# filrg/split_learning

Hardware: AMD Instinct MI355X
Metric: images/sec (whole node) VGG16/CIFAR10 cut=7 (higher is better)
Workload: dtype fp32; 1 GPU; model=VGG16_CIFAR10, global_batch=32, image=3x32x32, cut_layer=7, optimizer=SGD(lr=5e-4, momentum=0.5), control_count=1, mode=serial-recompute, parallelism=split2 x dp1

## Files before the change

### split_learning_amd/ops/csrc/wino.hip

```cpp
#include "torch_util.h"

namespace slk {

template <bool FLIP>
__global__ void wino_wt_kernel(const float* __restrict__ w,
                               float* __restrict__ U, int Cw0, int Cw1) {
  const long total = (long)Cw0 * Cw1;
  const long tstride = (long)gridDim.x * blockDim.x;
  for (long e = (long)blockIdx.x * blockDim.x + threadIdx.x; e < 4 * total;
       e += tstride) {
    const int a = (int)(e & 3);
    const long i = e >> 2;
    const int cols = FLIP ? Cw0 : Cw1;
    const int c = (int)(i % cols);
    const int r = (int)(i / cols);
    const int co = FLIP ? c : r;
    const int ci = FLIP ? r : c;
    float t[3];
    #pragma unroll
    for (int b = 0; b < 3; ++b) {
      const float g0 = w[(((long)co * Cw1 + ci) * 3 + (FLIP ? 2 : 0)) * 3 +
                         (FLIP ? 2 - b : b)];
      const float g1 = w[(((long)co * Cw1 + ci) * 3 + 1) * 3 +
                         (FLIP ? 2 - b : b)];
      const float g2 = w[(((long)co * Cw1 + ci) * 3 + (FLIP ? 0 : 2)) * 3 +
                         (FLIP ? 2 - b : b)];
      t[b] = a == 0 ? g0
           : a == 1 ? 0.5f * (g0 + g1 + g2)
           : a == 2 ? 0.5f * (g0 - g1 + g2)
           : g2;
    }
    U[((long)(a * 4 + 0) * total) + i] = t[0];
    U[((long)(a * 4 + 1) * total) + i] = 0.5f * (t[0] + t[1] + t[2]);
    U[((long)(a * 4 + 2) * total) + i] = 0.5f * (t[0] - t[1] + t[2]);
    U[((long)(a * 4 + 3) * total) + i] = t[2];
  }
}

__global__ void wino_in_kernel(const float* __restrict__ x,
                               float* __restrict__ V, int B, int Ci, int H,
                               int W, int tH, int tW, int pad, FastDiv d_T,
                               FastDiv d_thw, FastDiv d_tw) {
  const int T = B * tH * tW;
  const long total = (long)Ci * T;
  const long stride = (long)gridDim.x * blockDim.x;
  for (long i = (long)blockIdx.x * blockDim.x + threadIdx.x; i < total;
       i += stride) {
    const unsigned cc = d_T.div((unsigned)i);
    const unsigned t = d_T.mod((unsigned)i, cc);
    const unsigned b = d_thw.div(t);
    const unsigned rem = d_thw.mod(t, b);
    const unsigned th = d_tw.div(rem);
    const unsigned tw = d_tw.mod(rem, th);
    const int ih0 = (int)th * 2 - pad;
    const int iw0 = (int)tw * 2 - pad;
    const float* xp = x + ((long)b * Ci + cc) * H * W;
    float d[4][4];
    #pragma unroll
    for (int a = 0; a < 4; ++a) {
      const int ih = ih0 + a;
      const bool hv = (unsigned)ih < (unsigned)H;
      #pragma unroll
      for (int bb = 0; bb < 4; ++bb) {
        const int iw = iw0 + bb;
        const bool v = hv && (unsigned)iw < (unsigned)W;
        d[a][bb] = v ? xp[(long)ih * W + iw] : 0.f;
      }
    }
    float u[4][4];
    #pragma unroll
    for (int bb = 0; bb < 4; ++bb) {
      u[0][bb] = d[0][bb] - d[2][bb];
      u[1][bb] = d[1][bb] + d[2][bb];
      u[2][bb] = d[2][bb] - d[1][bb];
      u[3][bb] = d[1][bb] - d[3][bb];
    }
    #pragma unroll
    for (int a = 0; a < 4; ++a) {
      const float v0 = u[a][0] - u[a][2];
      const float v1 = u[a][1] + u[a][2];
      const float v2 = u[a][2] - u[a][1];
      const float v3 = u[a][1] - u[a][3];
      V[((long)(a * 4 + 0) * Ci + cc) * T + t] = v0;
      V[((long)(a * 4 + 1) * Ci + cc) * T + t] = v1;
      V[((long)(a * 4 + 2) * Ci + cc) * T + t] = v2;
      V[((long)(a * 4 + 3) * Ci + cc) * T + t] = v3;
    }
  }
}

__global__ void wino_out_kernel(const float* __restrict__ Mm,
                                float* __restrict__ y,
                                const float* __restrict__ bias, int B, int Co,
                                int OH, int OW, int tH, int tW, FastDiv d_T,
                                FastDiv d_thw, FastDiv d_tw) {
  const int T = B * tH * tW;
  const long total = (long)Co * T;
  const long stride = (long)gridDim.x * blockDim.x;
  for (long i = (long)blockIdx.x * blockDim.x + threadIdx.x; i < total;
       i += stride) {
    const unsigned co = d_T.div((unsigned)i);
    const unsigned t = d_T.mod((unsigned)i, co);
    const unsigned b = d_thw.div(t);
    const unsigned rem = d_thw.mod(t, b);
    const unsigned th = d_tw.div(rem);
    const unsigned tw = d_tw.mod(rem, th);
    float m[4][4];
    #pragma unroll
    for (int f = 0; f < 16; ++f)
      m[f >> 2][f & 3] = Mm[((long)f * Co + co) * T + t];
    float u[2][4];
    #pragma unroll
    for (int bb = 0; bb < 4; ++bb) {
      u[0][bb] = m[0][bb] + m[1][bb] + m[2][bb];
      u[1][bb] = m[1][bb] - m[2][bb] - m[3][bb];
    }
    const float bv = bias != nullptr ? bias[co] : 0.f;
    float* yp = y + ((long)b * Co + co) * OH * OW + (long)th * 2 * OW + tw * 2;
    yp[0] = u[0][0] + u[0][1] + u[0][2] + bv;
    yp[1] = u[0][1] - u[0][2] - u[0][3] + bv;
    yp[OW] = u[1][0] + u[1][1] + u[1][2] + bv;
    yp[OW + 1] = u[1][1] - u[1][2] - u[1][3] + bv;
  }
}

__global__ void wino_gyA_kernel(const float* __restrict__ gy,
                                float* __restrict__ Wg, int B, int Co, int OH,
                                int OW, int tH, int tW, FastDiv d_T,
                                FastDiv d_thw, FastDiv d_tw) {
  const int T = B * tH * tW;
  const long total = (long)Co * T;
  const long stride = (long)gridDim.x * blockDim.x;
  for (long i = (long)blockIdx.x * blockDim.x + threadIdx.x; i < total;
       i += stride) {
    const unsigned co = d_T.div((unsigned)i);
    const unsigned t = d_T.mod((unsigned)i, co);
    const unsigned b = d_thw.div(t);
    const unsigned rem = d_thw.mod(t, b);
    const unsigned th = d_tw.div(rem);
    const unsigned tw = d_tw.mod(rem, th);
    const float* gp = gy + ((long)b * Co + co) * OH * OW
                      + (long)th * 2 * OW + tw * 2;
    const float g00 = gp[0], g01 = gp[1], g10 = gp[OW], g11 = gp[OW + 1];
    float r0c0 = g00, r0c1 = g01;
    float r1c0 = g00 + g10, r1c1 = g01 + g11;
    float r2c0 = g00 - g10, r2c1 = g01 - g11;
    float r3c0 = -g10, r3c1 = -g11;
    #pragma unroll
    for (int a = 0; a < 4; ++a) {
      const float c0 = a == 0 ? r0c0 : a == 1 ? r1c0 : a == 2 ? r2c0 : r3c0;
      const float c1 = a == 0 ? r0c1 : a == 1 ? r1c1 : a == 2 ? r2c1 : r3c1;
      Wg[((long)(a * 4 + 0) * Co + co) * T + t] = c0;
      Wg[((long)(a * 4 + 1) * Co + co) * T + t] = c0 + c1;
      Wg[((long)(a * 4 + 2) * Co + co) * T + t] = c0 - c1;
      Wg[((long)(a * 4 + 3) * Co + co) * T + t] = -c1;
    }
  }
}

__global__ void wino_gw_kernel(const float* __restrict__ dU,
                               float* __restrict__ gw, int Co, int Ci) {
  const long total = (long)Co * Ci;
  const long stride = (long)gridDim.x * blockDim.x;
  for (long i = (long)blockIdx.x * blockDim.x + threadIdx.x; i < total;
       i += stride) {
    float u[4][4];
    #pragma unroll
    for (int f = 0; f < 16; ++f) u[f >> 2][f & 3] = dU[(long)f * total + i];
    float t[3][4];
    #pragma unroll
    for (int b = 0; b < 4; ++b) {
      t[0][b] = u[0][b] + 0.5f * (u[1][b] + u[2][b]);
      t[1][b] = 0.5f * (u[1][b] - u[2][b]);
      t[2][b] = 0.5f * (u[1][b] + u[2][b]) + u[3][b];
    }
    #pragma unroll
    for (int r = 0; r < 3; ++r) {
      gw[i * 9 + r * 3 + 0] = t[r][0] + 0.5f * (t[r][1] + t[r][2]);
      gw[i * 9 + r * 3 + 1] = 0.5f * (t[r][1] - t[r][2]);
      gw[i * 9 + r * 3 + 2] = 0.5f * (t[r][1] + t[r][2]) + t[r][3];
    }
  }
}

at::Tensor matmul_f32(const at::Tensor&, const at::Tensor&, bool, bool,
                      c10::optional<at::Tensor>, bool);

at::Tensor conv2d_wino(const at::Tensor& x, const at::Tensor& w,
                       c10::optional<at::Tensor> bias, int pad, bool flip) {
  TORCH_CHECK(x.is_cuda() && x.dim() == 4 && x.scalar_type() == at::kFloat);
  TORCH_CHECK(w.size(2) == 3 && w.size(3) == 3, "wino: 3x3 only");
  auto xc = x.contiguous();
  auto wc = w.contiguous();
  const int B = x.size(0), H = x.size(2), W = x.size(3);
  const int Co = flip ? w.size(1) : w.size(0);
  const int Ci = flip ? w.size(0) : w.size(1);
  TORCH_CHECK(x.size(1) == Ci, "wino: channel mismatch");
  const int OH = H + 2 * pad - 2, OW = W + 2 * pad - 2;
  TORCH_CHECK(OH % 2 == 0 && OW % 2 == 0, "wino: even output dims only");
  const int tH = OH / 2, tW = OW / 2;
  const int T = B * tH * tW;
  auto stream = c10::hip::getCurrentHIPStream().stream();

  auto U = at::empty({16, Co, Ci}, x.options());
  auto V = at::empty({16, Ci, T}, x.options());
  {
    const long tot = (long)Co * Ci * 4;
    const int grid = (int)std::min<long>((tot + 255) / 256, 4096);
    if (flip) {
      hipLaunchKernelGGL(wino_wt_kernel<true>, dim3(grid), dim3(256), 0,
                         stream, wc.data_ptr<float>(), U.data_ptr<float>(),
                         (int)w.size(0), (int)w.size(1));
    } else {
      hipLaunchKernelGGL(wino_wt_kernel<false>, dim3(grid), dim3(256), 0,
                         stream, wc.data_ptr<float>(), U.data_ptr<float>(),
                         (int)w.size(0), (int)w.size(1));
    }
  }
  {
    FastDiv d_T, d_thw, d_tw;
    d_T.init(T);
    d_thw.init(tH * tW);
    d_tw.init(tW);
    const long tot = (long)Ci * T;
    const int grid = (int)std::min<long>((tot + 255) / 256, 8192);
    hipLaunchKernelGGL(wino_in_kernel, dim3(grid), dim3(256), 0, stream,
                       xc.data_ptr<float>(), V.data_ptr<float>(), B, Ci, H, W,
                       tH, tW, pad, d_T, d_thw, d_tw);
  }
  auto Mm = matmul_f32(U, V, false, false, c10::nullopt, false);
  auto y = at::empty({B, Co, OH, OW}, x.options());
  {
    FastDiv d_T, d_thw, d_tw;
    d_T.init(T);
    d_thw.init(tH * tW);
    d_tw.init(tW);
    const long tot = (long)Co * T;
    const int grid = (int)std::min<long>((tot + 255) / 256, 8192);
    hipLaunchKernelGGL(wino_out_kernel, dim3(grid), dim3(256), 0, stream,
                       Mm.data_ptr<float>(), y.data_ptr<float>(),
                       bias.has_value() ? bias->data_ptr<float>() : nullptr,
                       B, Co, OH, OW, tH, tW, d_T, d_thw, d_tw);
  }
  return y;
}


constexpr int WF_CO = 32;
constexpr int WF_T = 32;
constexpr int WF_CK = 8;
constexpr int WF_ULD = WF_CO + 1;
constexpr int WF_VLD = WF_T + 1;

template <bool FLIP>
__global__ __launch_bounds__(256, 3) void wino_fused_kernel(
    const float* __restrict__ x, const float* __restrict__ w,
    const float* __restrict__ bias, float* __restrict__ y, int B, int Ci,
    int H, int W, int Co, int OH, int OW, int tH, int tW, int pad,
    int ci_per, int CW, FastDiv d_thw, FastDiv d_tw) {
  const int ci_begin = blockIdx.z * ci_per;
  const int ci_end = min(Ci, ci_begin + ci_per);
  __shared__ float Ul[16 * WF_CK * WF_ULD];
  __shared__ float Vl[16 * WF_CK * WF_VLD];

  const int T = B * tH * tW;
  const int co0 = blockIdx.y * WF_CO;
  const int t0 = blockIdx.x * WF_T;

  const int tid = threadIdx.x;
  const int lane = tid & 63;
  const int wid = tid >> 6;
  const int wco = (wid >> 1) * 16;
  const int wt = (wid & 1) * 16;
  const int frag_r = lane >> 4;
  const int frag_c = lane & 15;

  f32x4 acc[16];
  #pragma unroll
  for (int f = 0; f < 16; ++f) acc[f] = f32x4{};

  const int v_ci = tid >> 5;
  const int v_t = tid & 31;
  const int tg = t0 + v_t;
  const unsigned vb = d_thw.div((unsigned)tg);
  const unsigned vrem = d_thw.mod((unsigned)tg, vb);
  const unsigned vth = d_tw.div(vrem);
  const unsigned vtw = d_tw.mod(vrem, vth);
  const int ih0 = (int)vth * 2 - pad;
  const int iw0 = (int)vtw * 2 - pad;
  const long xplane = ((long)vb * Ci + v_ci) * H * W;
  const int w_co = tid >> 3;
  const int w_ci = tid & 7;

  float d[4][4];
  float wr[9];

  auto load_regs = [&](int ci0) {
    const float* xp = x + xplane + (long)ci0 * H * W;
    #pragma unroll
    for (int a = 0; a < 4; ++a) {
      const int ih = ih0 + a;
      const bool hv = (unsigned)ih < (unsigned)H;
      #pragma unroll
      for (int bb = 0; bb < 4; ++bb) {
        const int iw = iw0 + bb;
        const bool v = hv && (unsigned)iw < (unsigned)W;
        d[a][bb] = v ? xp[(long)ih * W + iw] : 0.f;
      }
    }
    const long wbase = FLIP
        ? ((long)(ci0 + w_ci) * CW + (co0 + w_co)) * 9
        : ((long)(co0 + w_co) * CW + (ci0 + w_ci)) * 9;
    #pragma unroll
    for (int k = 0; k < 9; ++k) wr[k] = w[wbase + (FLIP ? 8 - k : k)];
  };

  auto store_stage = [&]() {
    float u[4][4];
    #pragma unroll
    for (int bb = 0; bb < 4; ++bb) {
      u[0][bb] = d[0][bb] - d[2][bb];
      u[1][bb] = d[1][bb] + d[2][bb];
      u[2][bb] = d[2][bb] - d[1][bb];
      u[3][bb] = d[1][bb] - d[3][bb];
    }
    #pragma unroll
    for (int a = 0; a < 4; ++a) {
      Vl[((a * 4 + 0) * WF_CK + v_ci) * WF_VLD + v_t] = u[a][0] - u[a][2];
      Vl[((a * 4 + 1) * WF_CK + v_ci) * WF_VLD + v_t] = u[a][1] + u[a][2];
      Vl[((a * 4 + 2) * WF_CK + v_ci) * WF_VLD + v_t] = u[a][2] - u[a][1];
      Vl[((a * 4 + 3) * WF_CK + v_ci) * WF_VLD + v_t] = u[a][1] - u[a][3];
    }
    float t0[3], t1[3], t2[3], t3[3];
    #pragma unroll
    for (int bb = 0; bb < 3; ++bb) {
      const float g0 = wr[bb], g1 = wr[3 + bb], g2 = wr[6 + bb];
      t0[bb] = g0;
      t1[bb] = 0.5f * (g0 + g1 + g2);
      t2[bb] = 0.5f * (g0 - g1 + g2);
      t3[bb] = g2;
    }
    const float* tr[4] = {t0, t1, t2, t3};
    #pragma unroll
    for (int a = 0; a < 4; ++a) {
      const float* t = tr[a];
      Ul[((a * 4 + 0) * WF_CK + w_ci) * WF_ULD + w_co] = t[0];
      Ul[((a * 4 + 1) * WF_CK + w_ci) * WF_ULD + w_co] = 0.5f * (t[0] + t[1] + t[2]);
      Ul[((a * 4 + 2) * WF_CK + w_ci) * WF_ULD + w_co] = 0.5f * (t[0] - t[1] + t[2]);
      Ul[((a * 4 + 3) * WF_CK + w_ci) * WF_ULD + w_co] = t[2];
    }
  };

  load_regs(ci_begin);
  for (int ci0 = ci_begin; ci0 < ci_end; ci0 += WF_CK) {
    store_stage();
    __syncthreads();
    if (ci0 + WF_CK < ci_end) load_regs(ci0 + WF_CK);
    #pragma unroll
    for (int f = 0; f < 16; ++f) {
      #pragma unroll
      for (int kk = 0; kk < WF_CK / 4; ++kk) {
        const int kr = kk * 4 + frag_r;
        const float a = Ul[(f * WF_CK + kr) * WF_ULD + wco + frag_c];
        const float b = Vl[(f * WF_CK + kr) * WF_VLD + wt + frag_c];
        acc[f] = __builtin_amdgcn_mfma_f32_16x16x4f32(a, b, acc[f], 0, 0, 0);
      }
    }
    __syncthreads();
  }

  #pragma unroll
  for (int i = 0; i < 4; ++i) {
    const int co = co0 + wco + frag_r * 4 + i;
    const int t = t0 + wt + frag_c;
    if (co >= Co || t >= T) continue;
    float m[4][4];
    #pragma unroll
    for (int f = 0; f < 16; ++f) m[f >> 2][f & 3] = acc[f][i];
    float u0[4], u1[4];
    #pragma unroll
    for (int bb = 0; bb < 4; ++bb) {
      u0[bb] = m[0][bb] + m[1][bb] + m[2][bb];
      u1[bb] = m[1][bb] - m[2][bb] - m[3][bb];
    }
    const float bv = (bias != nullptr && blockIdx.z == 0) ? bias[co] : 0.f;
    const unsigned b = d_thw.div((unsigned)t);
    const unsigned rem = d_thw.mod((unsigned)t, b);
    const unsigned th = d_tw.div(rem);
    const unsigned tw = d_tw.mod(rem, th);
    float* yp = y + (long)blockIdx.z * B * Co * OH * OW +
                ((long)b * Co + co) * OH * OW + (long)th * 2 * OW + tw * 2;
    const float o00 = u0[0] + u0[1] + u0[2] + bv;
    const float o01 = u0[1] - u0[2] - u0[3] + bv;
    const float o10 = u1[0] + u1[1] + u1[2] + bv;
    const float o11 = u1[1] - u1[2] - u1[3] + bv;
    yp[0] = o00;
    yp[1] = o01;
    yp[OW] = o10;
    yp[OW + 1] = o11;
  }
}

at::Tensor conv2d_wino_bwdw(const at::Tensor& gy, const at::Tensor& x,
                            int pad) {
  TORCH_CHECK(gy.is_cuda() && x.is_cuda() && gy.dim() == 4 && x.dim() == 4);
  auto gyc = gy.contiguous();
  auto xc = x.contiguous();
  const int B = x.size(0), Ci = x.size(1), H = x.size(2), W = x.size(3);
  const int Co = gy.size(1), OH = gy.size(2), OW = gy.size(3);
  TORCH_CHECK(OH == H + 2 * pad - 2 && OW == W + 2 * pad - 2,
              "wino_bwdw geometry");
  TORCH_CHECK(OH % 2 == 0 && OW % 2 == 0, "wino_bwdw: even output dims only");
  const int tH = OH / 2, tW = OW / 2;
  const int T = B * tH * tW;
  auto stream = c10::hip::getCurrentHIPStream().stream();
  FastDiv d_T, d_thw, d_tw;
  d_T.init(T);
  d_thw.init(tH * tW);
  d_tw.init(tW);

  auto Wg = at::empty({16, Co, T}, x.options());
  auto Vx = at::empty({16, Ci, T}, x.options());
  {
    const long tot = (long)Co * T;
    const int grid = (int)std::min<long>((tot + 255) / 256, 8192);
    hipLaunchKernelGGL(wino_gyA_kernel, dim3(grid), dim3(256), 0, stream,
                       gyc.data_ptr<float>(), Wg.data_ptr<float>(), B, Co, OH,
                       OW, tH, tW, d_T, d_thw, d_tw);
  }
  {
    const long tot = (long)Ci * T;
    const int grid = (int)std::min<long>((tot + 255) / 256, 8192);
    hipLaunchKernelGGL(wino_in_kernel, dim3(grid), dim3(256), 0, stream,
                       xc.data_ptr<float>(), Vx.data_ptr<float>(), B, Ci, H, W,
                       tH, tW, pad, d_T, d_thw, d_tw);
  }
  auto dU = matmul_f32(Wg, Vx, false, true, c10::nullopt, false);
  auto gw = at::empty({Co, Ci, 3, 3}, x.options());
  {
    const long tot = (long)Co * Ci;
    const int grid = (int)std::min<long>((tot + 255) / 256, 4096);
    hipLaunchKernelGGL(wino_gw_kernel, dim3(grid), dim3(256), 0, stream,
                       dU.data_ptr<float>(), gw.data_ptr<float>(), Co, Ci);
  }
  return gw;
}

__global__ __launch_bounds__(256, 2) void wino_bwdw_fused_kernel(
    const float* __restrict__ gy, const float* __restrict__ x,
    float* __restrict__ slab, int B, int Ci, int H, int W, int Co, int OH,
    int OW, int tH, int tW, int pad, int t_per, FastDiv d_thw, FastDiv d_tw) {
  __shared__ float Gl[16 * 8 * 33];
  __shared__ float Xl[16 * 8 * 33];

  const int T = B * tH * tW;
  const int ci0 = blockIdx.y * 32;
  const int co0 = blockIdx.x * 32;
  const int t_begin = blockIdx.z * t_per;
  const int t_end = min(T, t_begin + t_per);

  const int tid = threadIdx.x;
  const int lane = tid & 63;
  const int wid = tid >> 6;
  const int wco = (wid >> 1) * 16;
  const int wci = (wid & 1) * 16;
  const int frag_r = lane >> 4;
  const int frag_c = lane & 15;

  f32x4 acc[16];
  #pragma unroll
  for (int f = 0; f < 16; ++f) acc[f] = f32x4{};

  const int s_ch = tid >> 3;
  const int s_t = tid & 7;

  float gg[2][2];
  float xd[4][4];

  auto load_regs = [&](int t0) {
    const int t = t0 + s_t;
    const int tc = t < T ? t : T - 1;
    const bool tv = t < t_end;
    const unsigned b = d_thw.div((unsigned)tc);
    const unsigned rem = d_thw.mod((unsigned)tc, b);
    const unsigned th = d_tw.div(rem);
    const unsigned tw = d_tw.mod(rem, th);
    {
      const float* gp = gy + ((long)b * Co + co0 + s_ch) * OH * OW
                        + (long)th * 2 * OW + tw * 2;
      gg[0][0] = tv ? gp[0] : 0.f;
      gg[0][1] = tv ? gp[1] : 0.f;
      gg[1][0] = tv ? gp[OW] : 0.f;
      gg[1][1] = tv ? gp[OW + 1] : 0.f;
    }
    {
      const int ih0 = (int)th * 2 - pad;
      const int iw0 = (int)tw * 2 - pad;
      const float* xp = x + ((long)b * Ci + ci0 + s_ch) * H * W;
      #pragma unroll
      for (int a = 0; a < 4; ++a) {
        const int ih = ih0 + a;
        const bool hv = tv && (unsigned)ih < (unsigned)H;
        #pragma unroll
        for (int bb = 0; bb < 4; ++bb) {
          const int iw = iw0 + bb;
          const bool v = hv && (unsigned)iw < (unsigned)W;
          xd[a][bb] = v ? xp[(long)ih * W + iw] : 0.f;
        }
      }
    }
  };

  auto store_stage = [&]() {
    const float r0c0 = gg[0][0], r0c1 = gg[0][1];
    const float r1c0 = gg[0][0] + gg[1][0], r1c1 = gg[0][1] + gg[1][1];
    const float r2c0 = gg[0][0] - gg[1][0], r2c1 = gg[0][1] - gg[1][1];
    const float r3c0 = -gg[1][0], r3c1 = -gg[1][1];
    #pragma unroll
    for (int a = 0; a < 4; ++a) {
      const float c0 = a == 0 ? r0c0 : a == 1 ? r1c0 : a == 2 ? r2c0 : r3c0;
      const float c1 = a == 0 ? r0c1 : a == 1 ? r1c1 : a == 2 ? r2c1 : r3c1;
      Gl[((a * 4 + 0) * 8 + s_t) * 33 + s_ch] = c0;
      Gl[((a * 4 + 1) * 8 + s_t) * 33 + s_ch] = c0 + c1;
      Gl[((a * 4 + 2) * 8 + s_t) * 33 + s_ch] = c0 - c1;
      Gl[((a * 4 + 3) * 8 + s_t) * 33 + s_ch] = -c1;
    }
    float u[4][4];
    #pragma unroll
    for (int bb = 0; bb < 4; ++bb) {
      u[0][bb] = xd[0][bb] - xd[2][bb];
      u[1][bb] = xd[1][bb] + xd[2][bb];
      u[2][bb] = xd[2][bb] - xd[1][bb];
      u[3][bb] = xd[1][bb] - xd[3][bb];
    }
    #pragma unroll
    for (int a = 0; a < 4; ++a) {
      Xl[((a * 4 + 0) * 8 + s_t) * 33 + s_ch] = u[a][0] - u[a][2];
      Xl[((a * 4 + 1) * 8 + s_t) * 33 + s_ch] = u[a][1] + u[a][2];
      Xl[((a * 4 + 2) * 8 + s_t) * 33 + s_ch] = u[a][2] - u[a][1];
      Xl[((a * 4 + 3) * 8 + s_t) * 33 + s_ch] = u[a][1] - u[a][3];
    }
  };

  load_regs(t_begin);
  for (int t0 = t_begin; t0 < t_end; t0 += 8) {
    store_stage();
    __syncthreads();
    if (t0 + 8 < t_end) load_regs(t0 + 8);
    #pragma unroll
    for (int f = 0; f < 16; ++f) {
      #pragma unroll
      for (int kk = 0; kk < 2; ++kk) {
        const int kr = kk * 4 + frag_r;
        const float a = Gl[(f * 8 + kr) * 33 + wco + frag_c];
        const float b = Xl[(f * 8 + kr) * 33 + wci + frag_c];
        acc[f] = __builtin_amdgcn_mfma_f32_16x16x4f32(a, b, acc[f], 0, 0, 0);
      }
    }
    __syncthreads();
  }

  const long numel = (long)Co * Ci * 9;
  #pragma unroll
  for (int i = 0; i < 4; ++i) {
    const int co = co0 + wco + frag_r * 4 + i;
    const int ci = ci0 + wci + frag_c;
    if (co >= Co || ci >= Ci) continue;
    float u[4][4];
    #pragma unroll
    for (int f = 0; f < 16; ++f) u[f >> 2][f & 3] = acc[f][i];
    float t3[3][4];
    #pragma unroll
    for (int bb = 0; bb < 4; ++bb) {
      t3[0][bb] = u[0][bb] + 0.5f * (u[1][bb] + u[2][bb]);
      t3[1][bb] = 0.5f * (u[1][bb] - u[2][bb]);
      t3[2][bb] = 0.5f * (u[1][bb] + u[2][bb]) + u[3][bb];
    }
    float* gp = slab + (long)blockIdx.z * numel + ((long)co * Ci + ci) * 9;
    #pragma unroll
    for (int r = 0; r < 3; ++r) {
      gp[r * 3 + 0] = t3[r][0] + 0.5f * (t3[r][1] + t3[r][2]);
      gp[r * 3 + 1] = 0.5f * (t3[r][1] - t3[r][2]);
      gp[r * 3 + 2] = 0.5f * (t3[r][1] + t3[r][2]) + t3[r][3];
    }
  }
}

at::Tensor conv2d_wino_bwdw_fused(const at::Tensor& gy, const at::Tensor& x,
                                  int pad) {
  TORCH_CHECK(gy.is_cuda() && x.is_cuda() && gy.dim() == 4 && x.dim() == 4);
  auto gyc = gy.contiguous();
  auto xc = x.contiguous();
  const int B = x.size(0), Ci = x.size(1), H = x.size(2), W = x.size(3);
  const int Co = gy.size(1), OH = gy.size(2), OW = gy.size(3);
  TORCH_CHECK(OH == H + 2 * pad - 2 && OW == W + 2 * pad - 2,
              "wino_bwdw_fused geometry");
  TORCH_CHECK(OH % 2 == 0 && OW % 2 == 0 && Co % 32 == 0 && Ci % 32 == 0,
              "wino_bwdw_fused shape requirements");
  const int tH = OH / 2, tW = OW / 2;
  const int T = B * tH * tW;
  auto stream = c10::hip::getCurrentHIPStream().stream();

  const long base_blocks = (long)(Co / 32) * (Ci / 32);
  int splits = 1;
  if (base_blocks < 256) {
    splits = (int)((256 + base_blocks - 1) / base_blocks);
    const int max_splits = (T + 7) / 8;
    if (splits > max_splits) splits = max_splits;
  }
  int t_per = ((T / splits + 7) / 8) * 8;
  if (t_per < 8) t_per = 8;
  splits = (T + t_per - 1) / t_per;

  auto slab = at::empty({splits, Co, Ci, 3, 3}, x.options());
  FastDiv d_thw, d_tw;
  d_thw.init(tH * tW);
  d_tw.init(tW);
  dim3 grid(Co / 32, Ci / 32, splits);
  hipLaunchKernelGGL(wino_bwdw_fused_kernel, grid, dim3(256), 0, stream,
                     gyc.data_ptr<float>(), xc.data_ptr<float>(),
                     slab.data_ptr<float>(), B, Ci, H, W, Co, OH, OW, tH, tW,
                     pad, t_per, d_thw, d_tw);
  if (splits == 1) {
    return slab.view({Co, Ci, 3, 3});
  }
  auto gw = at::empty({Co, Ci, 3, 3}, x.options());
  slab_reduce(slab.data_ptr<float>(), splits, gw.data_ptr<float>(), gw.numel(),
              stream);
  return gw;
}

at::Tensor conv2d_wino_fused(const at::Tensor& x, const at::Tensor& w,
                             c10::optional<at::Tensor> bias, int pad,
                             bool flip) {
  TORCH_CHECK(x.is_cuda() && x.dim() == 4 && x.scalar_type() == at::kFloat);
  TORCH_CHECK(w.size(2) == 3 && w.size(3) == 3, "wino_fused: 3x3 only");
  auto xc = x.contiguous();
  auto wc = w.contiguous();
  const int B = x.size(0), H = x.size(2), W = x.size(3);
  const int Co = flip ? w.size(1) : w.size(0);
  const int Ci = flip ? w.size(0) : w.size(1);
  TORCH_CHECK(x.size(1) == Ci, "wino_fused: channel mismatch");
  const int OH = H + 2 * pad - 2, OW = W + 2 * pad - 2;
  const int tH = OH / 2, tW = OW / 2;
  const int T = B * tH * tW;
  TORCH_CHECK(Co % 32 == 0 && T % 32 == 0 && Ci % 8 == 0 && OH % 2 == 0
              && OW % 2 == 0, "wino_fused shape requirements");
  auto stream = c10::hip::getCurrentHIPStream().stream();
  const int CW = (int)w.size(1);
  const long base_blocks = (long)(T / 32) * (Co / 32);
  int splits = 1;
  if (base_blocks < 256) {
    splits = (int)((256 + base_blocks - 1) / base_blocks);
    const int max_splits = Ci / WF_CK;
    if (splits > max_splits) splits = max_splits;
  }
  int ci_per = ((Ci / splits + WF_CK - 1) / WF_CK) * WF_CK;
  splits = (Ci + ci_per - 1) / ci_per;

  auto y = at::empty({B, Co, OH, OW}, x.options());
  at::Tensor slab;
  if (splits > 1) slab = at::empty({splits, B, Co, OH, OW}, x.options());
  float* yw = splits > 1 ? slab.data_ptr<float>() : y.data_ptr<float>();
  FastDiv d_thw, d_tw;
  d_thw.init(tH * tW);
  d_tw.init(tW);
  dim3 grid(T / 32, Co / 32, splits);
  if (flip) {
    hipLaunchKernelGGL(wino_fused_kernel<true>, grid, dim3(256), 0, stream,
                       xc.data_ptr<float>(), wc.data_ptr<float>(),
                       bias.has_value() ? bias->data_ptr<float>() : nullptr,
                       yw, B, Ci, H, W, Co, OH, OW, tH, tW,
                       pad, ci_per, CW, d_thw, d_tw);
  } else {
    hipLaunchKernelGGL(wino_fused_kernel<false>, grid, dim3(256), 0, stream,
                       xc.data_ptr<float>(), wc.data_ptr<float>(),
                       bias.has_value() ? bias->data_ptr<float>() : nullptr,
                       yw, B, Ci, H, W, Co, OH, OW, tH, tW,
                       pad, ci_per, CW, d_thw, d_tw);
  }
  if (splits > 1) {
    slab_reduce(slab.data_ptr<float>(), splits, y.data_ptr<float>(), y.numel(),
                stream);
  }
  return y;
}

}
```

Before: 13650 images/sec.

## Repack Winograd LDS tiles for 128-bit reads and software-pipelined MFMA k-steps

Changes the shared-memory layout of the transformed U/V (and G/X in the weight-gradient kernel) tiles so each row/channel holds its 16 Winograd components contiguously with padded strides. Stores and MFMA operand reads become 128-bit vector accesses, with operand loads prefetched one group ahead under a scheduling barrier. Weight loads in the forward kernel become two vector loads plus a scalar. The aim is to cut LDS instruction count and bank conflicts in the inner loop. The cost is higher shared-memory use, which may lower occupancy, and the weight vector loads may be unaligned.

```diff
diff --git a/split_learning_amd/ops/csrc/wino.hip b/split_learning_amd/ops/csrc/wino.hip
--- a/split_learning_amd/ops/csrc/wino.hip
+++ b/split_learning_amd/ops/csrc/wino.hip
@@ -249,8 +249,38 @@
 constexpr int WF_CO = 32;
 constexpr int WF_T = 32;
 constexpr int WF_CK = 8;
-constexpr int WF_ULD = WF_CO + 1;
-constexpr int WF_VLD = WF_T + 1;
+constexpr int WF_KS = 20;
+constexpr int WF_RS = 168;
+constexpr int WF_OP = 32 * WF_RS;
+
+__device__ __forceinline__ void wino_kstep_mfma(const float* pa,
+                                                const float* pb,
+                                                f32x4 (&acc)[16]) {
+  const f32x4* a0 = reinterpret_cast<const f32x4*>(pa);
+  const f32x4* a1 = reinterpret_cast<const f32x4*>(pa + 4 * WF_KS);
+  const f32x4* b0 = reinterpret_cast<const f32x4*>(pb);
+  const f32x4* b1 = reinterpret_cast<const f32x4*>(pb + 4 * WF_KS);
+  f32x4 ra0 = a0[0], rb0 = b0[0], ra1 = a1[0], rb1 = b1[0];
+  #pragma unroll
+  for (int g = 0; g < 4; ++g) {
+    const f32x4 ca0 = ra0, cb0 = rb0, ca1 = ra1, cb1 = rb1;
+    if (g < 3) {
+      ra0 = a0[g + 1];
+      rb0 = b0[g + 1];
+      ra1 = a1[g + 1];
+      rb1 = b1[g + 1];
+    }
+    __builtin_amdgcn_sched_barrier(0);
+    #pragma unroll
+    for (int j = 0; j < 4; ++j)
+      acc[g * 4 + j] = __builtin_amdgcn_mfma_f32_16x16x4f32(
+          ca0[j], cb0[j], acc[g * 4 + j], 0, 0, 0);
+    #pragma unroll
+    for (int j = 0; j < 4; ++j)
+      acc[g * 4 + j] = __builtin_amdgcn_mfma_f32_16x16x4f32(
+          ca1[j], cb1[j], acc[g * 4 + j], 0, 0, 0);
+  }
+}
 
 template <bool FLIP>
 __global__ __launch_bounds__(256, 3) void wino_fused_kernel(
@@ -260,8 +290,8 @@
     int ci_per, int CW, FastDiv d_thw, FastDiv d_tw) {
   const int ci_begin = blockIdx.z * ci_per;
   const int ci_end = min(Ci, ci_begin + ci_per);
-  __shared__ float Ul[16 * WF_CK * WF_ULD];
-  __shared__ float Vl[16 * WF_CK * WF_VLD];
+  __shared__ __attribute__((aligned(16))) float Ul[WF_OP];
+  __shared__ __attribute__((aligned(16))) float Vl[WF_OP];
 
   const int T = B * tH * tW;
   const int co0 = blockIdx.y * WF_CO;
@@ -293,7 +323,8 @@
   const int w_ci = tid & 7;
 
   float d[4][4];
-  float wr[9];
+  f32x4 wq0, wq1;
+  float w8;
 
   auto load_regs = [&](int ci0) {
     const float* xp = x + xplane + (long)ci0 * H * W;
@@ -311,8 +342,10 @@
     const long wbase = FLIP
         ? ((long)(ci0 + w_ci) * CW + (co0 + w_co)) * 9
         : ((long)(co0 + w_co) * CW + (ci0 + w_ci)) * 9;
-    #pragma unroll
-    for (int k = 0; k < 9; ++k) wr[k] = w[wbase + (FLIP ? 8 - k : k)];
+    using f32x4u = __attribute__((ext_vector_type(4), aligned(4))) float;
+    wq0 = *reinterpret_cast<const f32x4u*>(w + wbase);
+    wq1 = *reinterpret_cast<const f32x4u*>(w + wbase + 4);
+    w8 = w[wbase + 8];
   };
 
   auto store_stage = [&]() {
@@ -324,13 +357,17 @@
       u[2][bb] = d[2][bb] - d[1][bb];
       u[3][bb] = d[1][bb] - d[3][bb];
     }
+    f32x4* vp = reinterpret_cast<f32x4*>(&Vl[v_t * WF_RS + v_ci * WF_KS]);
     #pragma unroll
     for (int a = 0; a < 4; ++a) {
-      Vl[((a * 4 + 0) * WF_CK + v_ci) * WF_VLD + v_t] = u[a][0] - u[a][2];
-      Vl[((a * 4 + 1) * WF_CK + v_ci) * WF_VLD + v_t] = u[a][1] + u[a][2];
-      Vl[((a * 4 + 2) * WF_CK + v_ci) * WF_VLD + v_t] = u[a][2] - u[a][1];
-      Vl[((a * 4 + 3) * WF_CK + v_ci) * WF_VLD + v_t] = u[a][1] - u[a][3];
-    }
+      vp[a] = f32x4{u[a][0] - u[a][2], u[a][1] + u[a][2],
+                    u[a][2] - u[a][1], u[a][1] - u[a][3]};
+    }
+    const float raw[9] = {wq0[0], wq0[1], wq0[2], wq0[3], wq1[0],
+                          wq1[1], wq1[2], wq1[3], w8};
+    float wr[9];
+    #pragma unroll
+    for (int k = 0; k < 9; ++k) wr[k] = raw[FLIP ? 8 - k : k];
     float t0[3], t1[3], t2[3], t3[3];
     #pragma unroll
     for (int bb = 0; bb < 3; ++bb) {
@@ -341,31 +378,24 @@
       t3[bb] = g2;
     }
     const float* tr[4] = {t0, t1, t2, t3};
+    f32x4* up = reinterpret_cast<f32x4*>(&Ul[w_co * WF_RS + w_ci * WF_KS]);
     #pragma unroll
     for (int a = 0; a < 4; ++a) {
       const float* t = tr[a];
-      Ul[((a * 4 + 0) * WF_CK + w_ci) * WF_ULD + w_co] = t[0];
-      Ul[((a * 4 + 1) * WF_CK + w_ci) * WF_ULD + w_co] = 0.5f * (t[0] + t[1] + t[2]);
-      Ul[((a * 4 + 2) * WF_CK + w_ci) * WF_ULD + w_co] = 0.5f * (t[0] - t[1] + t[2]);
-      Ul[((a * 4 + 3) * WF_CK + w_ci) * WF_ULD + w_co] = t[2];
+      up[a] = f32x4{t[0], 0.5f * (t[0] + t[1] + t[2]),
+                    0.5f * (t[0] - t[1] + t[2]), t[2]};
     }
   };
+
+  const float* pa = &Ul[(wco + frag_c) * WF_RS + frag_r * WF_KS];
+  const float* pb = &Vl[(wt + frag_c) * WF_RS + frag_r * WF_KS];
 
   load_regs(ci_begin);
   for (int ci0 = ci_begin; ci0 < ci_end; ci0 += WF_CK) {
     store_stage();
     __syncthreads();
     if (ci0 + WF_CK < ci_end) load_regs(ci0 + WF_CK);
-    #pragma unroll
-    for (int f = 0; f < 16; ++f) {
-      #pragma unroll
-      for (int kk = 0; kk < WF_CK / 4; ++kk) {
-        const int kr = kk * 4 + frag_r;
-        const float a = Ul[(f * WF_CK + kr) * WF_ULD + wco + frag_c];
-        const float b = Vl[(f * WF_CK + kr) * WF_VLD + wt + frag_c];
-        acc[f] = __builtin_amdgcn_mfma_f32_16x16x4f32(a, b, acc[f], 0, 0, 0);
-      }
-    }
+    wino_kstep_mfma(pa, pb, acc);
     __syncthreads();
   }
 
@@ -450,8 +480,8 @@
     const float* __restrict__ gy, const float* __restrict__ x,
     float* __restrict__ slab, int B, int Ci, int H, int W, int Co, int OH,
     int OW, int tH, int tW, int pad, int t_per, FastDiv d_thw, FastDiv d_tw) {
-  __shared__ float Gl[16 * 8 * 33];
-  __shared__ float Xl[16 * 8 * 33];
+  __shared__ __attribute__((aligned(16))) float Gl[WF_OP];
+  __shared__ __attribute__((aligned(16))) float Xl[WF_OP];
 
   const int T = B * tH * tW;
   const int ci0 = blockIdx.y * 32;
@@ -516,14 +546,13 @@
     const float r1c0 = gg[0][0] + gg[1][0], r1c1 = gg[0][1] + gg[1][1];
     const float r2c0 = gg[0][0] - gg[1][0], r2c1 = gg[0][1] - gg[1][1];
     const float r3c0 = -gg[1][0], r3c1 = -gg[1][1];
+    f32x4* gp4 = reinterpret_cast<f32x4*>(&Gl[s_ch * WF_RS + s_t * WF_KS]);
+    f32x4* xp4 = reinterpret_cast<f32x4*>(&Xl[s_ch * WF_RS + s_t * WF_KS]);
     #pragma unroll
     for (int a = 0; a < 4; ++a) {
       const float c0 = a == 0 ? r0c0 : a == 1 ? r1c0 : a == 2 ? r2c0 : r3c0;
       const float c1 = a == 0 ? r0c1 : a == 1 ? r1c1 : a == 2 ? r2c1 : r3c1;
-      Gl[((a * 4 + 0) * 8 + s_t) * 33 + s_ch] = c0;
-      Gl[((a * 4 + 1) * 8 + s_t) * 33 + s_ch] = c0 + c1;
-      Gl[((a * 4 + 2) * 8 + s_t) * 33 + s_ch] = c0 - c1;
-      Gl[((a * 4 + 3) * 8 + s_t) * 33 + s_ch] = -c1;
+      gp4[a] = f32x4{c0, c0 + c1, c0 - c1, -c1};
     }
     float u[4][4];
     #pragma unroll
@@ -535,28 +564,20 @@
     }
     #pragma unroll
     for (int a = 0; a < 4; ++a) {
-      Xl[((a * 4 + 0) * 8 + s_t) * 33 + s_ch] = u[a][0] - u[a][2];
-      Xl[((a * 4 + 1) * 8 + s_t) * 33 + s_ch] = u[a][1] + u[a][2];
-      Xl[((a * 4 + 2) * 8 + s_t) * 33 + s_ch] = u[a][2] - u[a][1];
-      Xl[((a * 4 + 3) * 8 + s_t) * 33 + s_ch] = u[a][1] - u[a][3];
+      xp4[a] = f32x4{u[a][0] - u[a][2], u[a][1] + u[a][2],
+                     u[a][2] - u[a][1], u[a][1] - u[a][3]};
     }
   };
+
+  const float* pa = &Gl[(wco + frag_c) * WF_RS + frag_r * WF_KS];
+  const float* pb = &Xl[(wci + frag_c) * WF_RS + frag_r * WF_KS];
 
   load_regs(t_begin);
   for (int t0 = t_begin; t0 < t_end; t0 += 8) {
     store_stage();
     __syncthreads();
     if (t0 + 8 < t_end) load_regs(t0 + 8);
-    #pragma unroll
-    for (int f = 0; f < 16; ++f) {
-      #pragma unroll
-      for (int kk = 0; kk < 2; ++kk) {
-        const int kr = kk * 4 + frag_r;
-        const float a = Gl[(f * 8 + kr) * 33 + wco + frag_c];
-        const float b = Xl[(f * 8 + kr) * 33 + wci + frag_c];
-        acc[f] = __builtin_amdgcn_mfma_f32_16x16x4f32(a, b, acc[f], 0, 0, 0);
-      }
-    }
+    wino_kstep_mfma(pa, pb, acc);
     __syncthreads();
   }
 
```

Measured after the change: 14350 images/sec (median of 6 runs). 5.2% higher.
